# knowhunger/go-libp2p-pubsub

Hardware: AMD Instinct MI355X
Metric: peer-topic score updates/s + msg deliveries/s @1M peers, 1-8 GPUs, %HBM BW (higher is better)
Workload: dtype f64; 1 GPU; cfg3: 1M peers x 8 topics, full P1-P7 refreshScores()+score() per DecayInterval, connectSome d=6 overlay, spam-test topic params; peers_per_gpu=1000000, topics=8, pairs_per_gpu=11999954, records_per_gpu=95999632, parallelism=observers range-sharded, 1 shard(s), no exchange

## Files before the change

### go-libp2p-pubsub_amd/csrc/gsx_device.h

```cpp
#pragma once

#include <hip/hip_runtime.h>
#include <stdint.h>

namespace gsx {

struct DevTopicParams {
    double topic_weight;
    double w1, cap1;
    int64_t q1;
    double inv_q1;
    double w2, d2, cap2;
    double w3, d3, cap3, thr3;
    int64_t win3, act3;
    double w3b, d3b;
    double w4, d4;
    int32_t scored;
    int32_t pad;
};

__host__ __device__ __forceinline__ double q1_inverse(int64_t q1) { return q1 > 0 ? 1.0 / (double)q1 : 0.0; }

struct DevPeerParams {
    double topic_score_cap;
    double w5;
    double w6;
    int64_t thr6;
    double w7, thr7, d7;
    double decay_to_zero;
    int64_t retain_ns;
};

constexpr int KARG_TOPICS = 8;
struct KernParams {
    DevPeerParams pp;
    DevTopicParams tp[KARG_TOPICS];
};

constexpr int TILE = 64;
constexpr int NFIELD = 5;
enum Field { FMD = 0, MMD = 1, MFP = 2, IMD = 3, GRAFT = 4 };

__host__ __device__ __forceinline__ size_t rec_index(uint64_t p, uint32_t t, uint32_t n_topics, int field) {
    return (((p / TILE) * n_topics + t) * NFIELD + field) * TILE + (p % TILE);
}
__host__ __device__ __forceinline__ size_t flag_index(uint64_t p, uint32_t t, uint32_t n_topics) {
    return ((p / TILE) * n_topics + t) * TILE + (p % TILE);
}

constexpr uint8_t ZM_ZERO = 0, ZM_MAYBE = 1;
__host__ __device__ __forceinline__ size_t zmap_index(uint64_t p, uint32_t t, uint32_t n_topics, int field) {
    return ((p / TILE) * n_topics + t) * 2 + (size_t)(field - MFP);
}
__host__ __device__ __forceinline__ size_t zmap_bytes(uint64_t n_tiles, uint32_t n_topics) {
    return ((n_tiles * n_topics * 2 + 3) / 4 + 1) * 4;
}

constexpr int PZ_APP = 0, PZ_P6 = 1, PZ_ENTRY = 4;
__host__ __device__ __forceinline__ size_t pzmap_bytes(uint64_t n_tiles) { return (n_tiles + 1) * PZ_ENTRY; }

struct DevState {
    double* rec;
    uint8_t* rflags;
    uint8_t* zmap;
    uint8_t* pzmap;
    uint8_t* pflags;
    int64_t* expire;
    double* bp;
    double* app;
    const uint32_t* ipg;
    uint32_t* ipcount;
    double* score;
    const DevTopicParams* tp;
    uint64_t n_pairs;
    uint32_t n_topics;
    int64_t last_refresh;
    uint32_t phase;
    uint32_t wb_period;
    double decay_to_zero;
    double d7;
};

constexpr uint8_t REC_IN_MESH = 0x01;
constexpr uint8_t REC_ACTIVE = 0x02;
constexpr uint8_t REC_FRESH = 0x04;
constexpr uint8_t REC_EPOCH = 0x18;
constexpr int REC_EPOCH_SHIFT = 3;
constexpr uint8_t PAIR_PRESENT = 0x01;
constexpr uint8_t PAIR_CONNECTED = 0x02;
constexpr uint8_t PAIR_EPOCH = 0x0C;
constexpr int PAIR_EPOCH_SHIFT = 2;
constexpr uint32_t IPG_NONE = 0xFFFFFFFFu;
constexpr uint32_t IPG_WL = 0x80000000u;

struct DevEvent {
    uint32_t kind;
    uint32_t topic;
    uint64_t pair;
    int64_t now_ns;
    int64_t arg;
};

struct DevSynthSpec {
    uint64_t seed;
    int64_t now;
    double fmd_max, mmd_max, mfp_max, imd_max;
    double p_in_mesh;
    int64_t graft_window;
    double bp_max, p_disc, p_abs;
    int64_t expire_jitter;
    uint32_t sybil_first;
};

constexpr uint8_t EDGE_OUTBOUND = 0x01, EDGE_DIRECT = 0x02, EDGE_GOSSIPSUB = 0x04, EDGE_FLOODSUB = 0x08,
                  EDGE_NO_PX = 0x10;
constexpr uint32_t ROUTER_FLOODSUB = 0, ROUTER_GOSSIPSUB = 1, ROUTER_RANDOMSUB = 2;
constexpr uint32_t NO_PAIR = 0xFFFFFFFFu;
constexpr uint8_t FWD_FORWARD = 0x01;
constexpr uint8_t FWD_PUBLISH = 0x02;
constexpr uint8_t FWD_RSUB_CAND = 0x04;
constexpr uint8_t FWD_SEND = 0x07;
constexpr uint8_t FWD_GIN = 0x08;
constexpr int RANDOMSUB_D = 6;
constexpr int MAX_HOPS = 64;
enum {
    STAT_DUPS = 0,
    STAT_HOP0 = 1,
    STAT_EDGE_SENDS = STAT_HOP0 + MAX_HOPS + 1,
    STAT_NEW_WORDS,
    STAT_BACKSENDS,
    STAT_REJECTED,
    STAT_IGNORED,
    STAT_GRAY,
    STAT_HALO0,
    STAT_WORDS = STAT_HALO0 + MAX_HOPS + 1
};
constexpr uint32_t HALO = 0x80000000u;
constexpr uint32_t HALO_GRAY = 0x40000000u;
constexpr uint32_t HALO_SLOT = 0x3FFFFFFFu;
constexpr int PIN_FWD_SHIFT = 29;
constexpr uint32_t MAX_RANKS = 64;
constexpr uint32_t PIN_RDROP = 1u << 28;
constexpr uint32_t PIN_NODE_MASK = PIN_RDROP - 1;
// ... 735 lines not shown
```

### go-libp2p-pubsub_amd/csrc/gsx_engine.cpp

```cpp
#include <hip/hip_runtime.h>

#include <algorithm>
#include <map>
#include <atomic>
#include <chrono>
#include <array>
#include <cmath>
#include <cstdio>
#include <cstdlib>
#include <cstring>
#include <deque>
#include <functional>
#include <string>
#include <unordered_map>
#include <unordered_set>
#include <vector>

#include "../../include/gsx.h"
#include "gsx_device.h"

namespace {

constexpr int64_t kSecond = 1000000000LL;
constexpr int64_t kTimeCacheDuration = 120 * kSecond;
constexpr uint64_t kHostScoreMax = 1u << 16;

bool invalid_number(double x) { return std::isnan(x) || std::isinf(x); }

enum { kDeliveryUnknown = 0, kDeliveryValid, kDeliveryInvalid, kDeliveryIgnored, kDeliveryThrottled };

struct RecKey {
    uint32_t obs;
    uint64_t msg;
    bool operator==(const RecKey& o) const { return obs == o.obs && msg == o.msg; }
};
struct RecKeyHash {
    size_t operator()(const RecKey& k) const {
        uint64_t x = k.msg ^ (uint64_t(k.obs) * 0x9E3779B97F4A7C15ULL);
        x ^= x >> 31;
        x *= 0xbf58476d1ce4e5b9ULL;
        x ^= x >> 29;
        return size_t(x);
    }
};
struct DeliveryRecord {
    int status = kDeliveryUnknown;
    int64_t first_seen = 0;
    int64_t validated = 0;
    bool validated_set = false;
    std::vector<uint64_t> peers;
    bool peers_nil = false;
};

}

struct gsx_engine {
    int device = 0;
    hipStream_t stream = nullptr;
    hipEvent_t ev_start = nullptr, ev_stop = nullptr, ev_staged = nullptr;
    std::string err;

    uint32_t T = 0;
    gsx_peer_score_params pp{};
    bool pp_set = false;
    gsx_thresholds th{};
    gsx_topic_score_params tp[GSX_MAX_TOPICS]{};
    bool scored[GSX_MAX_TOPICS]{};
    gsx::DevTopicParams* d_tp = nullptr;

    bool loaded = false;
    uint32_t n_nodes = 0;
    uint64_t E = 0, rs = 0, n_tiles = 0;
    int64_t last_refresh = 0;
    uint32_t phase = 0;
    uint32_t wb_period = 4;
    bool retained_possible = false;
    int64_t retain_horizon = INT64_MIN;
    uint64_t purge_launches = 0;
    std::vector<int64_t> row_ptr;
    std::vector<int32_t> col_host;
    std::vector<uint32_t> pair_obs;
    std::vector<uint32_t> ipg_host;
    std::vector<uint32_t> group_ip;
    std::vector<uint8_t> ip_wl;
    uint32_t n_groups = 0;

    double* d_rec = nullptr;
    uint8_t* d_rflags = nullptr;
    uint8_t* d_zmap = nullptr;
    uint8_t* d_pzmap = nullptr;
    void* d_tmp = nullptr;
    uint32_t* d_nbad = nullptr;
    uint8_t *d_pflags = nullptr, *d_eflags = nullptr;
    int64_t* d_expire = nullptr;
    double *d_bp = nullptr, *d_app = nullptr, *d_score = nullptr;
    uint32_t *d_ipg = nullptr, *d_ipcount = nullptr;
    int32_t* d_col = nullptr;
    int64_t* d_row_ptr = nullptr;
    uint32_t* d_rev = nullptr;
    std::vector<uint8_t> eflags_host;
    bool floodsub_peers = true;
    int64_t max_deg = 0;

    gsx_gossipsub_params gp{};
    int64_t* d_backoff = nullptr;
    uint8_t* d_bo8 = nullptr;
    uint64_t *d_ctl = nullptr, *d_resp = nullptr;
    uint8_t* d_dirty = nullptr;
    uint32_t *d_long = nullptr, *d_nlong = nullptr;
    unsigned long long* d_hbstats = nullptr;
    uint32_t* d_rngk = nullptr;
    gsx::IhaveSlot* d_ihave_slot = nullptr;
    gsx::IhaveSlot* d_ihave_unit = nullptr;
    uint8_t* d_ihave_tag = nullptr;
    uint32_t *d_work = nullptr, *d_nwork = nullptr, *d_hubwork = nullptr, *d_hubs = nullptr;
    uint8_t* d_tcnt = nullptr;
    uint16_t* d_mcount = nullptr;
    std::vector<uint32_t> hubs_host;
    std::vector<uint8_t> gossip_prev;
    uint8_t* d_gelig = nullptr;
    uint32_t ihave_round = 0;
    bool have_gossip = false;
    bool hb_clean = false;
    bool hb_tracing = false;
    uint64_t* d_tr_acc = nullptr;
    uint64_t* d_tr_hp = nullptr;
    gsx::HbState hb{};
    bool hb_active = false;
// ... 420 lines not shown
#define HIPCHK(e, call)                                                                          \
    do {                                                                                         \
        hipError_t _st = (call);                                                                 \
        if (_st != hipSuccess)                                                                   \
            return fail((e), GSX_EDEVICE, std::string(#call ": ") + hipGetErrorString(_st));    \
    } while (0)

struct ZeroBatch {
    gsx_engine* e;
    gsx::ZeroSpans z{};
    explicit ZeroBatch(gsx_engine* e_) : e(e_) {}
    int add(void* p, size_t bytes) {
        if (!p || !bytes) return GSX_OK;
        if (z.k == gsx::ZERO_SPANS)
            if (int rc = flush()) return rc;
        z.p[z.k] = static_cast<uint8_t*>(p);
        z.n[z.k++] = bytes;
        return GSX_OK;
    }
    int flush() {
        if (!z.k) return GSX_OK;
        HIPCHK(e, gsx::launch_zero_spans(z, e->stream));
        z.k = 0;
        return GSX_OK;
    }
};

int gx_busy(gsx_engine* e) {
    if (e->gxr.pending) return fail(e, GSX_ESTATE, "a sharded gossip exchange is in flight: gsx_gx_end first");
    return GSX_OK;
}

gsx::DevState dev_state(const gsx_engine* e) {
    gsx::DevState s{};
    s.rec = e->d_rec;
    s.rflags = e->d_rflags;
    s.zmap = e->d_zmap;
    s.pzmap = e->d_pzmap;
    s.pflags = e->d_pflags;
    s.expire = e->d_expire;
    s.bp = e->d_bp;
    s.app = e->d_app;
    s.ipg = e->d_ipg;
    s.ipcount = e->d_ipcount;
    s.score = e->d_score;
    s.tp = e->d_tp;
    s.n_pairs = e->E;
    s.n_topics = e->T;
    s.last_refresh = e->last_refresh;
    s.phase = e->phase;
    s.wb_period = e->wb_period;
    s.decay_to_zero = e->pp.decay_to_zero;
    s.d7 = e->pp.behaviour_penalty_decay;
    return s;
}

constexpr int64_t kRetainUnknown = INT64_MAX;
void note_retained(gsx_engine* e, int64_t bound) {
    e->retained_possible = true;
    e->retain_horizon = std::max(e->retain_horizon, bound);
}
void note_retained_events(gsx_engine* e, const std::vector<gsx_event>& evs) {
    for (const gsx_event& x : evs)
        if (x.kind == GSX_EV_REMOVE_PEER)
            note_retained(e, (int64_t)((uint64_t)x.now_ns + (uint64_t)e->pp.retain_score_ns));
}

int pzmap_mark_p6(gsx_engine* e) {
    if (!e->loaded) return GSX_OK;
    HIPCHK(e, gsx::launch_pzmap_fill(dev_state(e), gsx::PZ_P6, gsx::ZM_MAYBE, e->stream));
    return GSX_OK;
}

gsx::DevEvent dev_event(const gsx_engine* e, const gsx_event& x) {
    if (x.kind == GSX_EV_ADD_PEER) {
        const uint32_t u = e->pair_obs[x.pair];
        return gsx::DevEvent{x.kind, x.topic, x.pair, e->row_ptr[u], e->row_ptr[u + 1]};
    }
    return gsx::DevEvent{x.kind, x.topic, x.pair, x.now_ns, x.arg};
}

int materialize_all(gsx_engine* e) {
    if (!e->loaded) return GSX_OK;
    HIPCHK(e, gsx::launch_materialize(dev_state(e), e->stream));
    e->phase = 0;
    return GSX_OK;
}

gsx::DevPeerParams dev_peer_params(const gsx_engine* e) {
    gsx::DevPeerParams d{};
    d.topic_score_cap = e->pp.topic_score_cap;
    d.w5 = e->pp.app_specific_weight;
    d.w6 = e->pp.ip_colocation_factor_weight;
    d.thr6 = e->pp.ip_colocation_factor_threshold;
    d.w7 = e->pp.behaviour_penalty_weight;
    d.thr7 = e->pp.behaviour_penalty_threshold;
    d.d7 = e->pp.behaviour_penalty_decay;
    d.decay_to_zero = e->pp.decay_to_zero;
    d.retain_ns = e->pp.retain_score_ns;
    return d;
}

gsx::DevTopicParams dev_topic_params(const gsx_engine* e, uint32_t t);

gsx::KernParams kern_params(const gsx_engine* e) {
    gsx::KernParams k{};
    k.pp = dev_peer_params(e);
    for (uint32_t t = 0; t < e->T && t < (uint32_t)gsx::KARG_TOPICS; ++t) k.tp[t] = dev_topic_params(e, t);
    return k;
}

gsx::DevTopicParams dev_topic_params(const gsx_engine* e, uint32_t t) {
    gsx::DevTopicParams d{};
    const gsx_topic_score_params& p = e->tp[t];
    d.topic_weight = p.topic_weight;
    d.w1 = p.time_in_mesh_weight;
    d.cap1 = p.time_in_mesh_cap;
    d.q1 = e->scored[t] ? p.time_in_mesh_quantum_ns : 1;
    d.inv_q1 = gsx::q1_inverse(d.q1);
    d.w2 = p.first_message_deliveries_weight;
    d.d2 = p.first_message_deliveries_decay;
    d.cap2 = p.first_message_deliveries_cap;
    d.w3 = p.mesh_message_deliveries_weight;
    d.d3 = p.mesh_message_deliveries_decay;
    d.cap3 = p.mesh_message_deliveries_cap;
    d.thr3 = p.mesh_message_deliveries_threshold;
    d.win3 = p.mesh_message_deliveries_window_ns;
    d.act3 = p.mesh_message_deliveries_activation_ns;
    d.w3b = p.mesh_failure_penalty_weight;
    d.d3b = p.mesh_failure_penalty_decay;
    d.w4 = p.invalid_message_deliveries_weight;
    d.d4 = p.invalid_message_deliveries_decay;
    d.scored = e->scored[t] ? 1 : 0;
    return d;
}

int upload_topic_params(gsx_engine* e) {
    gsx::DevTopicParams h[GSX_MAX_TOPICS]{};
    for (uint32_t t = 0; t < e->T; ++t) h[t] = dev_topic_params(e, t);
    HIPCHK(e, hipMemcpyAsync(e->d_tp, h, sizeof(gsx::DevTopicParams) * GSX_MAX_TOPICS, hipMemcpyHostToDevice,
                             e->stream));
    HIPCHK(e, hipStreamSynchronize(e->stream));
    return GSX_OK;
}

void seen_release(gsx_engine* e, uint64_t* p, size_t ) {
    if (!p) return;
    auto it = e->seen_cap.find(p);
    e->seen_pool.emplace_back(it != e->seen_cap.end() ? it->second : 0, p);
}
uint64_t* seen_acquire(gsx_engine* e, size_t words) {
    size_t best = e->seen_pool.size();
    for (size_t i = 0; i < e->seen_pool.size(); ++i)
        if (e->seen_pool[i].first >= words && (best == e->seen_pool.size() || e->seen_pool[i].first < e->seen_pool[best].first))
            best = i;
    if (best < e->seen_pool.size()) {
        uint64_t* p = e->seen_pool[best].second;
        e->seen_pool.erase(e->seen_pool.begin() + (long)best);
        return p;
    }
    constexpr size_t kSlab = 4, kSlabMaxBytes = 64ull << 20;
    const size_t w = (std::max<size_t>(words, 1) + 31) & ~(size_t)31;
    const size_t n = 8 * w <= kSlabMaxBytes ? kSlab : 1;
    uint64_t* p = nullptr;
    if (hipMalloc((void**)&p, 8 * w * n) != hipSuccess) {
        if (n == 1 || hipMalloc((void**)&p, 8 * w) != hipSuccess) return nullptr;
        e->pool_slabs.push_back(p);
        e->seen_cap[p] = w;
        return p;
    }
    e->pool_slabs.push_back(p);
    for (size_t k = 0; k < n; ++k) e->seen_cap[p + k * w] = w;
    for (size_t k = 1; k < n; ++k) e->seen_pool.emplace_back(w, p + k * w);
    return p;
}
void seen_pool_free(gsx_engine* e) {
    e->seen_pool.clear();
    e->small_pool.clear();
    e->seen_cap.clear();
    for (void* x : e->pool_slabs) (void)hipFree(x);
    e->pool_slabs.clear();
}
uint8_t* small_acquire(gsx_engine* e, size_t bytes, size_t* got) {
    for (size_t i = 0; i < e->small_pool.size(); ++i)
        if (e->small_pool[i].first >= bytes && e->small_pool[i].first <= 4 * bytes + 4096) {
            uint8_t* p = e->small_pool[i].second;
// ... 1454 lines not shown
    }
    return GSX_OK;
}

int gsx_gc_deliveries(gsx_engine* e, int64_t now) {
    if (!e) return GSX_EINVAL;
    for (auto it = e->rec_queue.begin(); it != e->rec_queue.end();) {
        auto& q = it->second;
        while (!q.empty() && now > q.front().second) {
            e->recs.erase(RecKey{it->first, q.front().first});
            q.pop_front();
        }
        it = q.empty() ? e->rec_queue.erase(it) : std::next(it);
    }
    return GSX_OK;
}

int gsx_num_delivery_records(gsx_engine* e, uint64_t* out) {
    if (!e || !out) return GSX_EINVAL;
    *out = e->recs.size();
    return GSX_OK;
}

int gsx_refresh(gsx_engine* e, int64_t now) {
    if (!e) return GSX_EINVAL;
    if (!e->loaded) return fail(e, GSX_ESTATE, "no overlay loaded");
    if (int rc = fold_deferred(e)) return rc;
    int rc = flush(e);
    if (rc) return rc;
    const gsx::DevState s = dev_state(e);
    if (e->retained_possible) {
        HIPCHK(e, gsx::launch_purge(s, now, e->stream));
        ++e->purge_launches;
        if (now > e->retain_horizon) {
            e->retained_possible = false;
            e->retain_horizon = INT64_MIN;
        }
    }
    const bool region = e->t_active && e->t_used < e->t_max;
    HIPCHK(e, hipEventRecord(region ? e->tev[2 * e->t_used] : e->ev_start, e->stream));
    HIPCHK(e, rescore_all(e, s, now, true));
    HIPCHK(e, hipEventRecord(region ? e->tev[2 * e->t_used + 1] : e->ev_stop, e->stream));
    if (region) ++e->t_used;
    e->timed = !region;
    e->scores_exact();
    e->state_changed();
    e->last_refresh = now;
    e->phase = e->phase + 1 >= e->wb_period ? 0 : e->phase + 1;
    return GSX_OK;
}

int gsx_set_decay_writeback(gsx_engine* e, uint32_t k) {
    if (!e) return GSX_EINVAL;
    if (k != 1 && k != 2 && k != 4) return fail(e, GSX_EINVAL, "decay write-back period must be 1, 2 or 4");
    if (int rc = gx_busy(e)) return rc;
    if (int rc = fold_deferred(e)) return rc;
    if (int rc = flush(e)) return rc;
    if (int rc = materialize_all(e)) return rc;
    e->wb_period = k;
    return GSX_OK;
}

int gsx_last_refresh_ms(gsx_engine* e, float* ms) {
    if (!e || !ms) return GSX_EINVAL;
    if (!e->timed) return fail(e, GSX_ESTATE, "no refresh timed yet");
    HIPCHK(e, hipEventSynchronize(e->ev_stop));
    HIPCHK(e, hipEventElapsedTime(ms, e->ev_start, e->ev_stop));
    return GSX_OK;
}

int gsx_timing_begin(gsx_engine* e, uint32_t max_launches) {
    if (!e || max_launches == 0) return GSX_EINVAL;
    while (e->tev.size() < 2 * (size_t)max_launches) {
        hipEvent_t ev;
        HIPCHK(e, hipEventCreate(&ev));
        e->tev.push_back(ev);
    }
    e->t_max = max_launches;
    e->t_used = 0;
    e->t_active = true;
    return GSX_OK;
}

int gsx_timing_end(gsx_engine* e, double* total_ms, double* min_ms, double* max_ms, uint32_t* n) {
    if (!e || !total_ms || !n) return GSX_EINVAL;
    if (!e->t_active) return fail(e, GSX_ESTATE, "gsx_timing_begin not called");
    e->t_active = false;
    double sum = 0, lo = 0, hi = 0;
    for (uint32_t i = 0; i < e->t_used; ++i) {
        HIPCHK(e, hipEventSynchronize(e->tev[2 * i + 1]));
        float ms = 0;
        HIPCHK(e, hipEventElapsedTime(&ms, e->tev[2 * i], e->tev[2 * i + 1]));
        sum += ms;
        lo = i == 0 ? ms : std::min(lo, (double)ms);
        hi = i == 0 ? ms : std::max(hi, (double)ms);
    }
    *total_ms = sum;
    *n = e->t_used;
    if (min_ms) *min_ms = lo;
    if (max_ms) *max_ms = hi;
    return GSX_OK;
}

int gsx_scores(gsx_engine* e, double* out, size_t n) {
    if (!e || (n && !out)) return GSX_EINVAL;
    if (!e->loaded) return fail(e, GSX_ESTATE, "no overlay loaded");
    if (n != e->E) return fail(e, GSX_EINVAL, "score buffer size != pairs");
// ... 5022 lines not shown
```

### go-libp2p-pubsub_amd/csrc/gsx_kernels.hip

```cpp
#include "gsx_ops.h"

namespace gsx {


__device__ __forceinline__ uint64_t wave_uniform(uint64_t x) {
    return (uint64_t)__builtin_amdgcn_readfirstlane((uint32_t)x) |
           (uint64_t)__builtin_amdgcn_readfirstlane((uint32_t)(x >> 32)) << 32;
}

constexpr uint32_t ZM_MFP_BITS = 0x00FFu, ZM_IMD_BITS = 0xFF00u;
__device__ __forceinline__ uint32_t zmap_pair(const uint8_t* zmap, uint64_t o) {
    const uint32_t w = reinterpret_cast<const uint32_t*>(zmap)[o >> 2];
    return __builtin_amdgcn_readfirstlane((w >> ((uint32_t)(o & 2) * 8)) & 0xFFFFu);
}

template <int TT, bool REFRESH>
__global__ __launch_bounds__(256) void k_refresh_score(DevState s, KernParams kp, int64_t now,
                                                       const uint8_t* __restrict__ only,
                                                       const uint8_t* __restrict__ only2,
                                                       const unsigned long long* __restrict__ gate) {
    const uint64_t p = (uint64_t)blockIdx.x * 256u + threadIdx.x;
    if (p >= s.n_pairs) return;
    if (!REFRESH && gate && gate[0] + gate[1] == 0) return;
    if (!REFRESH && only && (!only[p] || (only2 && !only2[p]))) return;
    const int T = TT > 0 ? TT : (int)s.n_topics;
    const uint64_t lane = p % TILE;
    const uint64_t wtile = wave_uniform(p / TILE);
    const uint64_t zoff = wtile * (uint64_t)T * 2;
    uint32_t zm[TT > 0 ? TT : 1];
    if constexpr (TT > 0) {
#pragma unroll
        for (int t = 0; t < TT; ++t) zm[t] = zmap_pair(s.zmap, zoff + 2 * t);
    }
    const uint32_t pz = __builtin_amdgcn_readfirstlane(reinterpret_cast<const uint32_t*>(s.pzmap)[wtile]);
    const bool app_maybe = (pz >> (8 * PZ_APP)) & 0xFFu;
    const bool p6_maybe = !REFRESH || ((pz >> (8 * PZ_P6)) & 0xFFu);
    const uint8_t st = s.pflags[p];
    if (!(st & PAIR_PRESENT)) {
        s.score[p] = 0.0;
        return;
    }
    const DevPeerParams& pp = kp.pp;
    double p5 = 0.0;
    if (app_maybe) p5 = s.app[p];
    const bool conn = REFRESH && (st & PAIR_CONNECTED);
    const uint32_t phase = s.phase;
    const bool wb = REFRESH && phase + 1 >= s.wb_period;
    const bool lag = st & PAIR_CONNECTED;
    const uint8_t keep_conn = (uint8_t)~(REC_FRESH | (wb ? REC_EPOCH : 0));
    double* const tile = s.rec + (p / TILE) * (uint64_t)T * (NFIELD * TILE) + lane;
    uint8_t* const ftile = s.rflags + (p / TILE) * (uint64_t)T * TILE + lane;
    double score = 0.0;
    auto topic_step = [&](int t, const DevTopicParams& tp, double fmd, double mmd, double mfp, double imd,
                          int64_t graft, uint8_t fl, uint32_t zmt) {
        double* const r = tile + (uint64_t)t * (NFIELD * TILE);
        const double fmd0 = fmd, mmd0 = mmd, mfp0 = mfp, imd0 = imd;
        const uint32_t nd = (lag ? (phase - ((uint32_t)fl >> REC_EPOCH_SHIFT)) & 3u : 0u) + (conn ? 1u : 0u);
        const uint32_t nd0 = __builtin_amdgcn_readfirstlane(nd);
        auto decay_all = [&]() {
            fmd = decay(fmd, tp.d2, pp.decay_to_zero);
            mmd = decay(mmd, tp.d3, pp.decay_to_zero);
            mfp = decay(mfp, tp.d3b, pp.decay_to_zero);
            imd = decay(imd, tp.d4, pp.decay_to_zero);
        };
        if (__ballot(nd != nd0) == 0) {
            for (uint32_t i = 0; i < nd0; ++i) decay_all();
        } else {
            for (uint32_t i = 0; i < nd; ++i) decay_all();
        }
        if (wb) {
            if (conn && __double_as_longlong(fmd) != __double_as_longlong(fmd0)) __builtin_nontemporal_store(fmd, r + FMD * TILE);
            if (conn && __double_as_longlong(mmd) != __double_as_longlong(mmd0)) __builtin_nontemporal_store(mmd, r + MMD * TILE);
            if (conn && __double_as_longlong(mfp) != __double_as_longlong(mfp0)) __builtin_nontemporal_store(mfp, r + MFP * TILE);
            if (conn && __double_as_longlong(imd) != __double_as_longlong(imd0)) __builtin_nontemporal_store(imd, r + IMD * TILE);
        }
        const bool in_mesh = fl & REC_IN_MESH;
        int64_t mt = 0;
        if (conn) {
            mt = in_mesh ? now - graft : 0;
            const uint8_t nf = (uint8_t)((fl & keep_conn) | ((in_mesh && mt > tp.act3) ? REC_ACTIVE : 0));
            if (nf != fl) ftile[t * TILE] = nf;
            fl = nf;
        } else if (in_mesh && !(fl & REC_FRESH)) {
            mt = s.last_refresh - graft;
        }
        if constexpr (REFRESH) {
            if (zmt && __ballot(1) == ~0ull) {
                uint8_t* const zb = s.zmap + zoff + 2 * t;
                const bool z3 = (zmt & ZM_MFP_BITS) && __ballot(__double_as_longlong(mfp) != 0) == 0;
                const bool z4 = (zmt & ZM_IMD_BITS) && __ballot(__double_as_longlong(imd) != 0) == 0;
                if (z3 && !wb && __double_as_longlong(mfp0) != 0) r[MFP * TILE] = 0.0;
                if (z4 && !wb && __double_as_longlong(imd0) != 0) r[IMD * TILE] = 0.0;
                if (z3 && lane == 0) zb[0] = ZM_ZERO;
                if (z4 && lane == 0) zb[1] = ZM_ZERO;
            }
        }
        score += topic_score(tp, fl, mt, fmd, mmd, mfp, imd);
    };
    if constexpr (TT > 0) {
        double fmd[TT], mmd[TT], mfp[TT], imd[TT];
        int64_t gr[TT];
        uint8_t fl[TT];
#pragma unroll
        for (int t = 0; t < TT; ++t) {
            if (!kp.tp[t].scored) continue;
            const double* const r = tile + (uint64_t)t * (NFIELD * TILE);
            fmd[t] = __builtin_nontemporal_load(r + FMD * TILE);
            mmd[t] = __builtin_nontemporal_load(r + MMD * TILE);
            mfp[t] = (zm[t] & ZM_MFP_BITS) ? __builtin_nontemporal_load(r + MFP * TILE) : 0.0;
            imd[t] = (zm[t] & ZM_IMD_BITS) ? __builtin_nontemporal_load(r + IMD * TILE) : 0.0;
            fl[t] = ftile[t * TILE];
            gr[t] = (TT > 1 || (fl[t] & REC_IN_MESH))
                        ? __builtin_nontemporal_load(reinterpret_cast<const int64_t*>(r) + GRAFT * TILE)
                        : 0;
        }
#pragma unroll
        for (int t = 0; t < TT; ++t) {
            if (!kp.tp[t].scored) continue;
            topic_step(t, kp.tp[t], fmd[t], mmd[t], mfp[t], imd[t], gr[t], fl[t], zm[t]);
        }
    } else {
        for (int t = 0; t < T; ++t) {
            const DevTopicParams& tp = s.tp[t];
            if (!tp.scored) continue;
            const double* const r = tile + (uint64_t)t * (NFIELD * TILE);
            const uint32_t zmt = zmap_pair(s.zmap, zoff + 2 * t);
            const uint8_t fl = ftile[t * TILE];
            const int64_t graft = (fl & REC_IN_MESH) ? reinterpret_cast<const int64_t*>(r)[GRAFT * TILE] : 0;
            const double fmd = __builtin_nontemporal_load(r + FMD * TILE), mmd = __builtin_nontemporal_load(r + MMD * TILE);
            const double mfp = (zmt & ZM_MFP_BITS) ? __builtin_nontemporal_load(r + MFP * TILE) : 0.0;
            const double imd = (zmt & ZM_IMD_BITS) ? __builtin_nontemporal_load(r + IMD * TILE) : 0.0;
            topic_step(t, tp, fmd, mmd, mfp, imd, graft, fl, zmt);
        }
    }
    const double bp0 = s.bp[p];
    double bp = bp0;
    const uint32_t nb = (lag ? (phase - ((uint32_t)st >> PAIR_EPOCH_SHIFT)) & 3u : 0u) + (conn ? 1u : 0u);
    const uint32_t nb0 = __builtin_amdgcn_readfirstlane(nb);
    if (__ballot(nb != nb0) == 0) {
        for (uint32_t i = 0; i < nb0; ++i) bp = decay(bp, pp.d7, pp.decay_to_zero);
    } else {
        for (uint32_t i = 0; i < nb; ++i) bp = decay(bp, pp.d7, pp.decay_to_zero);
    }
    if (wb && conn) {
        if (__double_as_longlong(bp) != __double_as_longlong(bp0)) s.bp[p] = bp;
        if (st & PAIR_EPOCH) s.pflags[p] = st & ~PAIR_EPOCH;
    }
    double p6 = 0.0;
    const bool p6_read = pp.w6 != 0.0 && p6_maybe;
    if (p6_read) p6 = ip_colocation(s, pp, p);
    s.score[p] = score_tail_vals(pp, score, p5, p6, bp);
    if constexpr (REFRESH) {
        if ((app_maybe || p6_read) && __ballot(1) == ~0ull) {
            uint8_t* const pzb = s.pzmap + wtile * PZ_ENTRY;
            const bool z5 = app_maybe && __ballot(__double_as_longlong(p5) != 0) == 0;
            const bool z6 = p6_read && __ballot(__double_as_longlong(p6) != 0) == 0;
            if (z5 && lane == 0) pzb[PZ_APP] = ZM_ZERO;
            if (z6 && lane == 0) pzb[PZ_P6] = ZM_ZERO;
        }
    }
}

__global__ __launch_bounds__(256) void k_purge(DevState s, int64_t now) {
    const uint64_t p = (uint64_t)blockIdx.x * 256u + threadIdx.x;
    if (p >= s.n_pairs) return;
    const uint8_t st = s.pflags[p];
    if ((st & (PAIR_PRESENT | PAIR_CONNECTED)) != PAIR_PRESENT) return;
    if (!(now > s.expire[p])) return;
    s.pflags[p] = 0;
    const uint2 g = reinterpret_cast<const uint2*>(s.ipg)[p];
    if (g.x != IPG_NONE) atomicSub(&s.ipcount[g.x & ~IPG_WL], 1u);
    if (g.y != IPG_NONE && g.y != g.x) atomicSub(&s.ipcount[g.y & ~IPG_WL], 1u);
}


__device__ __forceinline__ void apply_event(const DevState& s, const DevPeerParams& pp, const DevEvent& e) {
    switch (e.kind) {
    case 1: ev_add_peer(s, pp, e.pair, (uint64_t)e.now_ns, (uint64_t)e.arg); break;
    case 2: ev_remove_peer(s, pp, e.pair, e.now_ns); break;
    case 3: ev_graft(s, e.pair, e.topic, e.now_ns); break;
    case 4: ev_prune(s, e.pair, e.topic); break;
    case 5: ev_first(s, e.pair, e.topic); break;
    case 6: ev_mesh(s, e.pair, e.topic); break;
    case 7: ev_invalid(s, e.pair, e.topic); break;
    case 8: ev_penalty(s, e.pair, e.arg); break;
    case 9:
        if (e.arg != 0) pzmap_mark(s, e.pair, PZ_APP);
        s.app[e.pair] = __longlong_as_double((long long)e.arg);
        break;
    default: break;
    }
}

__global__ __launch_bounds__(64) void k_apply_events(DevState s, DevPeerParams pp, const DevEvent* __restrict__ ev,
                                                     const uint32_t* __restrict__ group_off, uint32_t n_groups) {
// ... 278 lines not shown
hipError_t launch_mark_rows(const int64_t* row_ptr, const uint32_t* obs, uint32_t n, uint8_t* mask, uint8_t val,
                            hipStream_t st) {
    if (n == 0) return hipSuccess;
    hipLaunchKernelGGL(k_mark_rows, dim3(std::min<uint32_t>((n + 3) / 4, 4096)), dim3(256), 0, st, row_ptr, obs, n, mask,
                       val);
    return hipGetLastError();
}

hipError_t launch_apply_events(const DevState& s, const DevPeerParams& pp, const DevEvent* ev,
                               const uint32_t* group_off, uint32_t n_groups, hipStream_t st) {
    if (n_groups == 0) return hipSuccess;
    hipLaunchKernelGGL(k_apply_events, dim3(blocks_for(n_groups, 64)), dim3(64), 0, st, s, pp, ev, group_off,
                       n_groups);
    return hipGetLastError();
}

hipError_t launch_dropin(const DevState& s, const DevPeerParams& pp, const DevEvent* ev, const uint32_t* goff,
                         uint32_t n_groups, const uint32_t* obs, uint32_t n_obs, const uint64_t* prs, uint32_t n_prs,
                         const int64_t* row_ptr, double* hscore, uint32_t* flag, uint32_t tag, hipStream_t st) {
    hipLaunchKernelGGL(k_dropin, dim3(1), dim3(n_obs ? 1024 : 256), 0, st, s, pp, ev, goff, n_groups, obs, n_obs, prs,
                       n_prs, row_ptr, hscore, flag, tag);
    return hipGetLastError();
}

hipError_t launch_gather_scores(const double* score, const uint64_t* pairs, uint64_t n, double* out, hipStream_t st) {
    if (n == 0) return hipSuccess;
    const uint64_t b = (n + 255) / 256;
    hipLaunchKernelGGL(k_gather_scores, dim3((unsigned)(b < 4096 ? b : 4096)), dim3(256), 0, st, score, pairs, n, out);
    return hipGetLastError();
}

hipError_t launch_recap(const DevState& s, uint32_t topic, double cap2, double cap3, hipStream_t st) {
    if (s.n_pairs == 0) return hipSuccess;
    hipLaunchKernelGGL(k_recap, dim3(blocks_for(s.n_pairs, 256)), dim3(256), 0, st, s, topic, cap2, cap3);
    return hipGetLastError();
}

__global__ __launch_bounds__(256) void k_materialize(DevState s) {
    const uint64_t p = (uint64_t)blockIdx.x * 256u + threadIdx.x;
    const uint32_t t = blockIdx.y;
    if (p >= s.n_pairs) return;
    const size_t fi = flag_index(p, t, s.n_topics);
    const uint8_t fl = s.rflags[fi];
    const uint32_t k = rec_pend(s, s.pflags[p], fl, s.tp[t]);
    if (k) rec_store_decayed(s, p, t, k);
    if (fl & REC_EPOCH) s.rflags[fi] = fl & ~REC_EPOCH;
}
__global__ __launch_bounds__(256) void k_materialize_pairs(DevState s) {
    const uint64_t p = (uint64_t)blockIdx.x * 256u + threadIdx.x;
    if (p >= s.n_pairs) return;
    const uint8_t st = s.pflags[p];
    const uint32_t k = bp_pend(s, st);
    if (k) {
        const double o = s.bp[p], v = bp_decay(o, s.d7, s.decay_to_zero, k);
        if (__double_as_longlong(v) != __double_as_longlong(o)) s.bp[p] = v;
    }
    if (st & PAIR_EPOCH) s.pflags[p] = st & ~PAIR_EPOCH;
}
hipError_t launch_materialize(const DevState& s, hipStream_t st) {
    if (s.n_pairs == 0) return hipSuccess;
    hipLaunchKernelGGL(k_materialize, dim3(blocks_for(s.n_pairs, 256), s.n_topics), dim3(256), 0, st, s);
    hipLaunchKernelGGL(k_materialize_pairs, dim3(blocks_for(s.n_pairs, 256)), dim3(256), 0, st, s);
    return hipGetLastError();
}

__global__ __launch_bounds__(256) void k_pair_export(DevState s, uint8_t* __restrict__ pf, double* __restrict__ bp) {
    const uint64_t p = (uint64_t)blockIdx.x * 256u + threadIdx.x;
    if (p >= s.n_pairs) return;
    const uint8_t st = s.pflags[p];
    if (pf) pf[p] = st & ~PAIR_EPOCH;
    if (bp) bp[p] = bp_read(s, p, st);
}
hipError_t launch_pair_export(const DevState& s, uint8_t* pflags, double* bp, hipStream_t st) {
    if (s.n_pairs == 0) return hipSuccess;
    hipLaunchKernelGGL(k_pair_export, dim3(blocks_for(s.n_pairs, 256)), dim3(256), 0, st, s, pflags, bp);
    return hipGetLastError();
}

hipError_t launch_rebuild_ipcount(const DevState& s, uint32_t n_groups_ip, hipStream_t st) {
    hipError_t e = hipMemsetAsync(s.ipcount, 0, sizeof(uint32_t) * (n_groups_ip ? n_groups_ip : 1), st);
    if (e != hipSuccess || s.n_pairs == 0) return e;
    hipLaunchKernelGGL(k_rebuild_ipcount, dim3(blocks_for(s.n_pairs, 256)), dim3(256), 0, st, s);
    return hipGetLastError();
}

hipError_t launch_synthesize(const DevState& s, const int32_t* col, const DevSynthSpec& spec, hipStream_t st) {
    if (s.n_pairs == 0) return hipSuccess;
    const unsigned nb = blocks_for(s.n_pairs, 256);
    hipLaunchKernelGGL(k_synth_records, dim3(nb, s.n_topics), dim3(256), 0, st, s, col, spec);
    hipLaunchKernelGGL(k_synth_pairs, dim3(nb), dim3(256), 0, st, s, spec);
    return hipGetLastError();
}

hipError_t launch_tile_field(const DevState& s, int field, const void* src, hipStream_t st) {
    if (s.n_pairs == 0) return hipSuccess;
    hipLaunchKernelGGL(k_tile_field, dim3(blocks_for(s.n_pairs, 256), s.n_topics), dim3(256), 0, st, s, field, src);
    return hipGetLastError();
}

hipError_t launch_untile_field(const DevState& s, int field, void* dst, hipStream_t st) {
    if (s.n_pairs == 0) return hipSuccess;
    hipLaunchKernelGGL(k_untile_field, dim3(blocks_for(s.n_pairs, 256), s.n_topics), dim3(256), 0, st, s, field, dst);
    return hipGetLastError();
}

hipError_t launch_mesh_time_export(const DevState& s, int64_t* dst, hipStream_t st) {
    if (s.n_pairs == 0) return hipSuccess;
// ... 52 lines not shown
```

### go-libp2p-pubsub_amd/csrc/gsx_ops.h

```cpp
#pragma once

#include "gsx_device.h"

namespace gsx {


__device__ __forceinline__ double ip_colocation(const DevState& s, const DevPeerParams& pp, uint64_t p) {
    const uint2 g = reinterpret_cast<const uint2*>(s.ipg)[p];
    double result = 0.0;
    const uint32_t gs[2] = {g.x, g.y};
#pragma unroll
    for (int k = 0; k < 2; ++k) {
        const uint32_t id = gs[k];
        if (id == IPG_NONE || (id & IPG_WL)) continue;
        const int64_t peers_in_ip = (int64_t)s.ipcount[id];
        if (peers_in_ip > pp.thr6) {
            const double surpluss = (double)(peers_in_ip - pp.thr6);
            result += surpluss * surpluss;
        }
    }
    return result;
}

__device__ __forceinline__ double score_tail_vals(const DevPeerParams& pp, double score, double p5, double p6,
// ... 18 lines not shown
constexpr int64_t DIV_Q1_BOUND = 1ll << 50;

__host__ __device__ __forceinline__ int64_t div_q1(int64_t mt, int64_t q1, double inv) {
    if (inv != 0.0 && (uint64_t)mt + (uint64_t)DIV_Q1_BOUND - 1u < 2u * (uint64_t)DIV_Q1_BOUND - 1u) {
        const double est = (double)mt * inv;
        const double sum = est + 6755399441055744.0;
#if defined(__HIP_DEVICE_COMPILE__)
        const uint64_t bits = (uint64_t)__double_as_longlong(sum);
#else
        uint64_t bits;
        __builtin_memcpy(&bits, &sum, sizeof bits);
#endif
        int64_t n = (int64_t)(bits & ((1ull << 52) - 1)) - (1ll << 51);
        const int64_t r = (int64_t)((uint64_t)mt - (uint64_t)n * (uint64_t)q1);
        const bool neg = mt < 0;
        const bool up = neg ? r > 0 : r >= q1;
        const bool down = neg ? r <= -q1 : r < 0;
        n += (int64_t)up - (int64_t)down;
        return n;
    }
    return mt / q1;
}

__device__ __forceinline__ double topic_score(const DevTopicParams& tp, uint8_t fl, int64_t mesh_time, double fmd,
                                              double mmd, double mfp, double imd) {
    double ts = 0.0;
    if (fl & REC_IN_MESH) {
        double p1 = (double)div_q1(mesh_time, tp.q1, tp.inv_q1);
        if (p1 > tp.cap1) p1 = tp.cap1;
        ts += p1 * tp.w1;
    }
    const double p2 = fmd;
    ts += p2 * tp.w2;
    if (fl & REC_ACTIVE) {
        if (mmd < tp.thr3) {
            const double deficit = tp.thr3 - mmd;
            const double p3 = deficit * deficit;
            ts += p3 * tp.w3;
        }
    }
    const double p3b = mfp;
    ts += p3b * tp.w3b;
    const double p4 = (imd * imd);
    ts += p4 * tp.w4;
    return ts * tp.topic_weight;
}

__device__ __forceinline__ int64_t mesh_time_of(const DevState& s, uint8_t fl, uint64_t p, uint32_t t) {
    if (!(fl & REC_IN_MESH) || (fl & REC_FRESH)) return 0;
    const int64_t graft = reinterpret_cast<const int64_t*>(s.rec)[rec_index(p, t, s.n_topics, GRAFT)];
    return s.last_refresh - graft;
}

__device__ __forceinline__ double decay(double x, double d, double dtz) {
    x *= d;
    return x < dtz ? 0.0 : x;
}

__device__ __forceinline__ void zmap_mark(const DevState& s, uint64_t p, uint32_t t, int field) {
    s.zmap[zmap_index(p, t, s.n_topics, field)] = ZM_MAYBE;
}

__device__ __forceinline__ void pzmap_mark(const DevState& s, uint64_t p, int which) {
    s.pzmap[(p / TILE) * PZ_ENTRY + which] = ZM_MAYBE;
}
__device__ __forceinline__ void pzmap_mark_row(const DevState& s, uint64_t lo, uint64_t hi) {
    if (hi > s.n_pairs) hi = s.n_pairs;
    if (lo >= hi) return;
    for (uint64_t tile = lo / TILE; tile <= (hi - 1) / TILE; ++tile) s.pzmap[tile * PZ_ENTRY + PZ_P6] = ZM_MAYBE;
}

struct RecVals {
    double fmd, mmd, mfp, imd;
};

__device__ __forceinline__ uint32_t rec_pend(const DevState& s, uint8_t st, uint8_t fl, const DevTopicParams& tp) {
    return ((st & PAIR_CONNECTED) && tp.scored) ? ((s.phase - ((uint32_t)fl >> REC_EPOCH_SHIFT)) & 3u) : 0u;
}

__device__ __forceinline__ void rec_decay(RecVals& v, const DevTopicParams& tp, double dtz, uint32_t k) {
    for (uint32_t i = 0; i < k; ++i) {
        v.fmd = decay(v.fmd, tp.d2, dtz);
        v.mmd = decay(v.mmd, tp.d3, dtz);
        v.mfp = decay(v.mfp, tp.d3b, dtz);
        v.imd = decay(v.imd, tp.d4, dtz);
    }
}

__device__ __forceinline__ RecVals rec_read(const DevState& s, uint64_t p, uint32_t t, uint8_t st, uint8_t fl) {
    const size_t b = rec_index(p, t, s.n_topics, FMD);
    RecVals v = {s.rec[b + FMD * TILE], s.rec[b + MMD * TILE], s.rec[b + MFP * TILE], s.rec[b + IMD * TILE]};
    rec_decay(v, s.tp[t], s.decay_to_zero, rec_pend(s, st, fl, s.tp[t]));
    return v;
}
__device__ __forceinline__ RecVals rec_read(const DevState& s, uint64_t p, uint32_t t) {
    return rec_read(s, p, t, s.pflags[p], s.rflags[flag_index(p, t, s.n_topics)]);
}

__device__ __forceinline__ void rec_store_decayed(const DevState& s, uint64_t p, uint32_t t, uint32_t k) {
    const size_t b = rec_index(p, t, s.n_topics, FMD);
    const RecVals o = {s.rec[b + FMD * TILE], s.rec[b + MMD * TILE], s.rec[b + MFP * TILE], s.rec[b + IMD * TILE]};
    RecVals v = o;
    rec_decay(v, s.tp[t], s.decay_to_zero, k);
    if (__double_as_longlong(v.fmd) != __double_as_longlong(o.fmd)) s.rec[b + FMD * TILE] = v.fmd;
    if (__double_as_longlong(v.mmd) != __double_as_longlong(o.mmd)) s.rec[b + MMD * TILE] = v.mmd;
    if (__double_as_longlong(v.mfp) != __double_as_longlong(o.mfp)) {
        if (__double_as_longlong(v.mfp) != 0) zmap_mark(s, p, t, MFP);
        s.rec[b + MFP * TILE] = v.mfp;
    }
    if (__double_as_longlong(v.imd) != __double_as_longlong(o.imd)) {
        if (__double_as_longlong(v.imd) != 0) zmap_mark(s, p, t, IMD);
        s.rec[b + IMD * TILE] = v.imd;
    }
}

__device__ __forceinline__ uint8_t rec_materialize(const DevState& s, uint64_t p, uint32_t t, uint8_t st) {
    const size_t fi = flag_index(p, t, s.n_topics);
    const uint8_t fl = s.rflags[fi];
    const uint32_t k = rec_pend(s, st, fl, s.tp[t]);
    if (k) rec_store_decayed(s, p, t, k);
    const uint8_t nf = (uint8_t)((fl & ~REC_EPOCH) | (s.phase << REC_EPOCH_SHIFT));
    if (nf != fl) s.rflags[fi] = nf;
    return nf;
}
__device__ __forceinline__ uint8_t rec_materialize(const DevState& s, uint64_t p, uint32_t t) {
    return rec_materialize(s, p, t, s.pflags[p]);
}

__device__ __forceinline__ uint32_t bp_pend(const DevState& s, uint8_t st) {
    return (st & PAIR_CONNECTED) ? ((s.phase - ((uint32_t)st >> PAIR_EPOCH_SHIFT)) & 3u) : 0u;
}

__device__ __forceinline__ double bp_decay(double bp, double d7, double dtz, uint32_t k) {
    for (uint32_t i = 0; i < k; ++i) bp = decay(bp, d7, dtz);
    return bp;
}

__device__ __forceinline__ double bp_read(const DevState& s, uint64_t p, uint8_t st) {
    return bp_decay(s.bp[p], s.d7, s.decay_to_zero, bp_pend(s, st));
}

__device__ __forceinline__ uint8_t bp_materialize(const DevState& s, uint64_t p, uint8_t st) {
    if (!(st & PAIR_CONNECTED)) return st;
    const uint32_t k = bp_pend(s, st);
    if (k) {
        const double o = s.bp[p], v = bp_decay(o, s.d7, s.decay_to_zero, k);
        if (__double_as_longlong(v) != __double_as_longlong(o)) s.bp[p] = v;
    }
    const uint8_t nf = (uint8_t)((st & ~PAIR_EPOCH) | ((s.phase & 3u) << PAIR_EPOCH_SHIFT));
    if (nf != st) s.pflags[p] = nf;
    return nf;
}

__device__ __forceinline__ double eval_pair(const DevState& s, const DevPeerParams& pp, uint64_t p) {
    const uint8_t st = s.pflags[p];
    if (!(st & PAIR_PRESENT)) return 0.0;
    double score = 0.0;
    for (uint32_t t = 0; t < s.n_topics; ++t) {
        const DevTopicParams& tp = s.tp[t];
        if (!tp.scored) continue;
        const uint8_t fl = s.rflags[flag_index(p, t, s.n_topics)];
        const RecVals v = rec_read(s, p, t, st, fl);
        score += topic_score(tp, fl, mesh_time_of(s, fl, p, t), v.fmd, v.mmd, v.mfp, v.imd);
    }
    return score_tail(s, pp, p, score, bp_read(s, p, st));
}

__device__ __forceinline__ double add_ones_capped(double x, uint32_t k, double cap) {
    while (k && !(x >= 1.0 && x < 4503599627370496.0)) {
        x = x + 1;
        --k;
        if (x > cap) return cap;
    }
    while (k) {
        const unsigned long long bits = (unsigned long long)__double_as_longlong(x);
        const double top = __longlong_as_double((long long)((((bits >> 52) & 0x7FF) + 1) << 52));
        const double gap = top - x;
        const double s = ceil(gap) - 1;
        if (s >= (double)k) {
            x = x + (double)k;
            k = 0;
        } else {
            x = x + s;
            k -= (uint32_t)s;
            x = x + 1;
            --k;
        }
        if (x > cap) return cap;
        if (!(x < 4503599627370496.0))
            while (k) {
                x = x + 1;
                --k;
                if (x > cap) return cap;
            }
    }
    return x > cap ? cap : x;
}


__device__ __forceinline__ void ipcount_add(const DevState& s, uint64_t p, int delta) {
    const uint2 g = reinterpret_cast<const uint2*>(s.ipg)[p];
    if (g.x != IPG_NONE) s.ipcount[g.x & ~IPG_WL] += (uint32_t)delta;
    if (g.y != IPG_NONE && g.y != g.x) s.ipcount[g.y & ~IPG_WL] += (uint32_t)delta;
}

__device__ __forceinline__ bool scored_topic(const DevState& s, uint64_t p, uint32_t topic) {
    return (s.pflags[p] & PAIR_PRESENT) && topic < s.n_topics && s.tp[topic].scored;
}

__device__ inline void ev_add_peer(const DevState& s, const DevPeerParams& pp, uint64_t p, uint64_t row_lo,
                                   uint64_t row_hi) {
    const uint8_t st = s.pflags[p];
    const uint8_t ep = (uint8_t)(s.phase << REC_EPOCH_SHIFT);
    if (!(st & PAIR_PRESENT)) {
        for (uint32_t t = 0; t < s.n_topics; ++t) {
            const size_t b = rec_index(p, t, s.n_topics, FMD);
            for (int f = 0; f < NFIELD; ++f) s.rec[b + f * TILE] = 0.0;
            s.rflags[flag_index(p, t, s.n_topics)] = ep;
        }
        s.bp[p] = 0.0;
        s.expire[p] = 0;
        ipcount_add(s, p, +1);
        const uint2 g = reinterpret_cast<const uint2*>(s.ipg)[p];
        const bool over_x = g.x != IPG_NONE && !(g.x & IPG_WL) && (int64_t)s.ipcount[g.x] > pp.thr6;
        const bool over_y = g.y != IPG_NONE && !(g.y & IPG_WL) && (int64_t)s.ipcount[g.y] > pp.thr6;
        if (over_x || over_y) {
            pzmap_mark(s, p, PZ_P6);
            pzmap_mark_row(s, row_lo, row_hi);
        }
    } else if (!(st & PAIR_CONNECTED)) {
        for (uint32_t t = 0; t < s.n_topics; ++t) {
            const size_t fi = flag_index(p, t, s.n_topics);
            const uint8_t fl = s.rflags[fi];
            if ((fl & REC_EPOCH) != ep) s.rflags[fi] = (uint8_t)((fl & ~REC_EPOCH) | ep);
        }
    }
    if (!(st & PAIR_PRESENT) || !(st & PAIR_CONNECTED))
        s.pflags[p] = (uint8_t)(PAIR_PRESENT | PAIR_CONNECTED | ((s.phase & 3u) << PAIR_EPOCH_SHIFT));
}

__device__ inline void ev_remove_peer(const DevState& s, const DevPeerParams& pp, uint64_t p, int64_t now) {
    const uint8_t st = s.pflags[p];
    if (!(st & PAIR_PRESENT)) return;
    if (eval_pair(s, pp, p) > 0) {
        ipcount_add(s, p, -1);
        bp_materialize(s, p, st);
        s.pflags[p] = 0;
        return;
    }
    for (uint32_t t = 0; t < s.n_topics; ++t) {
        const DevTopicParams& tp = s.tp[t];
        if (!tp.scored) continue;
        const size_t b = rec_index(p, t, s.n_topics, FMD);
        const size_t fi = flag_index(p, t, s.n_topics);
        const uint8_t fl = rec_materialize(s, p, t, st);
        s.rec[b + FMD * TILE] = 0.0;
        const double threshold = tp.thr3;
        const double mmd = s.rec[b + MMD * TILE];
        if ((fl & REC_IN_MESH) && (fl & REC_ACTIVE) && mmd < threshold) {
            const double deficit = threshold - mmd;
            zmap_mark(s, p, t, MFP);
            s.rec[b + MFP * TILE] = s.rec[b + MFP * TILE] + deficit * deficit;
        }
        s.rflags[fi] = fl & ~(REC_IN_MESH | REC_FRESH);
    }
    bp_materialize(s, p, st);
    s.pflags[p] = PAIR_PRESENT;
    s.expire[p] = now + pp.retain_ns;
}

__device__ inline void ev_graft(const DevState& s, uint64_t p, uint32_t topic, int64_t now) {
    if (!scored_topic(s, p, topic)) return;
    reinterpret_cast<int64_t*>(s.rec)[rec_index(p, topic, s.n_topics, GRAFT)] = now;
    const size_t fi = flag_index(p, topic, s.n_topics);
    s.rflags[fi] = (uint8_t)((s.rflags[fi] & REC_EPOCH) | REC_IN_MESH | REC_FRESH);
}

__device__ inline void ev_prune(const DevState& s, uint64_t p, uint32_t topic) {
    if (!scored_topic(s, p, topic)) return;
    const size_t b = rec_index(p, topic, s.n_topics, FMD);
    const size_t fi = flag_index(p, topic, s.n_topics);
    const uint8_t fl = rec_materialize(s, p, topic);
    const double threshold = s.tp[topic].thr3;
    const double mmd = s.rec[b + MMD * TILE];
    if ((fl & REC_ACTIVE) && mmd < threshold) {
        const double deficit = threshold - mmd;
        zmap_mark(s, p, topic, MFP);
        s.rec[b + MFP * TILE] = s.rec[b + MFP * TILE] + deficit * deficit;
    }
    s.rflags[fi] = fl & ~(REC_IN_MESH | REC_FRESH);
}
// ... 104 lines not shown
```

Measured before the change: 145.9 billion peer-topic score updates/s.

## Widen decay epoch to 16 phases and chain multiplies before the zero threshold

Widens the per-record and per-pair epoch fields from 2 to 4 bits and raises the default write-back period from 4 to 16. Decayed counters are therefore written back to HBM less often, cutting store traffic during refresh. When every decay factor is in (0,1) and decay_to_zero is positive, pending decays are applied as a run of multiplies with a single threshold check at the end instead of one clamp per step. The chained form may differ from per-step clamping in edge cases, and lagging records now replay up to 16 decay steps when read.

```diff
diff --git a/go-libp2p-pubsub_amd/csrc/gsx_device.h b/go-libp2p-pubsub_amd/csrc/gsx_device.h
--- a/go-libp2p-pubsub_amd/csrc/gsx_device.h
+++ b/go-libp2p-pubsub_amd/csrc/gsx_device.h
@@ -16,7 +16,7 @@
     double w3b, d3b;
     double w4, d4;
     int32_t scored;
-    int32_t pad;
+    int32_t chain_ok;
 };
 
 __host__ __device__ __forceinline__ double q1_inverse(int64_t q1) { return q1 > 0 ? 1.0 / (double)q1 : 0.0; }
@@ -29,7 +29,11 @@
     double w7, thr7, d7;
     double decay_to_zero;
     int64_t retain_ns;
-};
+    int32_t dtz_ok;
+    int32_t bp_chain_ok;
+};
+
+__host__ __device__ __forceinline__ bool decay_chain_ok(double d, double dtz) { return d > 0.0 && d < 1.0 && dtz > 0.0; }
 
 constexpr int KARG_TOPICS = 8;
 struct KernParams {
@@ -79,16 +83,20 @@
     uint32_t wb_period;
     double decay_to_zero;
     double d7;
+    uint32_t dtz_ok;
+    uint32_t bp_chain_ok;
 };
 
 constexpr uint8_t REC_IN_MESH = 0x01;
 constexpr uint8_t REC_ACTIVE = 0x02;
 constexpr uint8_t REC_FRESH = 0x04;
-constexpr uint8_t REC_EPOCH = 0x18;
+constexpr uint32_t MAX_WB_PERIOD = 16;
+constexpr uint32_t EPOCH_MASK = MAX_WB_PERIOD - 1;
+constexpr uint8_t REC_EPOCH = 0x78;
 constexpr int REC_EPOCH_SHIFT = 3;
 constexpr uint8_t PAIR_PRESENT = 0x01;
 constexpr uint8_t PAIR_CONNECTED = 0x02;
-constexpr uint8_t PAIR_EPOCH = 0x0C;
+constexpr uint8_t PAIR_EPOCH = 0x3C;
 constexpr int PAIR_EPOCH_SHIFT = 2;
 constexpr uint32_t IPG_NONE = 0xFFFFFFFFu;
 constexpr uint32_t IPG_WL = 0x80000000u;
diff --git a/go-libp2p-pubsub_amd/csrc/gsx_engine.cpp b/go-libp2p-pubsub_amd/csrc/gsx_engine.cpp
--- a/go-libp2p-pubsub_amd/csrc/gsx_engine.cpp
+++ b/go-libp2p-pubsub_amd/csrc/gsx_engine.cpp
@@ -73,7 +73,7 @@
     uint64_t E = 0, rs = 0, n_tiles = 0;
     int64_t last_refresh = 0;
     uint32_t phase = 0;
-    uint32_t wb_period = 4;
+    uint32_t wb_period = gsx::MAX_WB_PERIOD;
     bool retained_possible = false;
     int64_t retain_horizon = INT64_MIN;
     uint64_t purge_launches = 0;
@@ -600,6 +600,8 @@
     s.wb_period = e->wb_period;
     s.decay_to_zero = e->pp.decay_to_zero;
     s.d7 = e->pp.behaviour_penalty_decay;
+    s.dtz_ok = e->pp.decay_to_zero > 0 ? 1u : 0u;
+    s.bp_chain_ok = gsx::decay_chain_ok(s.d7, s.decay_to_zero) ? 1u : 0u;
     return s;
 }
 
@@ -646,6 +648,8 @@
     d.d7 = e->pp.behaviour_penalty_decay;
     d.decay_to_zero = e->pp.decay_to_zero;
     d.retain_ns = e->pp.retain_score_ns;
+    d.dtz_ok = d.decay_to_zero > 0 ? 1 : 0;
+    d.bp_chain_ok = gsx::decay_chain_ok(d.d7, d.decay_to_zero) ? 1 : 0;
     return d;
 }
 
@@ -680,6 +684,7 @@
     d.w4 = p.invalid_message_deliveries_weight;
     d.d4 = p.invalid_message_deliveries_decay;
     d.scored = e->scored[t] ? 1 : 0;
+    d.chain_ok = (d.d2 > 0 && d.d2 < 1 && d.d3 > 0 && d.d3 < 1 && d.d3b > 0 && d.d3b < 1 && d.d4 > 0 && d.d4 < 1) ? 1 : 0;
     return d;
 }
 
@@ -2240,7 +2245,8 @@
 
 int gsx_set_decay_writeback(gsx_engine* e, uint32_t k) {
     if (!e) return GSX_EINVAL;
-    if (k != 1 && k != 2 && k != 4) return fail(e, GSX_EINVAL, "decay write-back period must be 1, 2 or 4");
+    if (k != 1 && k != 2 && k != 4 && k != gsx::MAX_WB_PERIOD)
+        return fail(e, GSX_EINVAL, "decay write-back period must be 1, 2, 4 or 16");
     if (int rc = gx_busy(e)) return rc;
     if (int rc = fold_deferred(e)) return rc;
     if (int rc = flush(e)) return rc;
diff --git a/go-libp2p-pubsub_amd/csrc/gsx_kernels.hip b/go-libp2p-pubsub_amd/csrc/gsx_kernels.hip
--- a/go-libp2p-pubsub_amd/csrc/gsx_kernels.hip
+++ b/go-libp2p-pubsub_amd/csrc/gsx_kernels.hip
@@ -55,19 +55,16 @@
                           int64_t graft, uint8_t fl, uint32_t zmt) {
         double* const r = tile + (uint64_t)t * (NFIELD * TILE);
         const double fmd0 = fmd, mmd0 = mmd, mfp0 = mfp, imd0 = imd;
-        const uint32_t nd = (lag ? (phase - ((uint32_t)fl >> REC_EPOCH_SHIFT)) & 3u : 0u) + (conn ? 1u : 0u);
+        const uint32_t nd = (lag ? (phase - ((uint32_t)fl >> REC_EPOCH_SHIFT)) & EPOCH_MASK : 0u) + (conn ? 1u : 0u);
         const uint32_t nd0 = __builtin_amdgcn_readfirstlane(nd);
-        auto decay_all = [&]() {
-            fmd = decay(fmd, tp.d2, pp.decay_to_zero);
-            mmd = decay(mmd, tp.d3, pp.decay_to_zero);
-            mfp = decay(mfp, tp.d3b, pp.decay_to_zero);
-            imd = decay(imd, tp.d4, pp.decay_to_zero);
-        };
+        const bool chain = tp.chain_ok && pp.dtz_ok;
+        RecVals v = {fmd, mmd, mfp, imd};
         if (__ballot(nd != nd0) == 0) {
-            for (uint32_t i = 0; i < nd0; ++i) decay_all();
+            rec_decay(v, tp, pp.decay_to_zero, nd0, chain);
         } else {
-            for (uint32_t i = 0; i < nd; ++i) decay_all();
-        }
+            rec_decay(v, tp, pp.decay_to_zero, nd, chain);
+        }
+        fmd = v.fmd, mmd = v.mmd, mfp = v.mfp, imd = v.imd;
         if (wb) {
             if (conn && __double_as_longlong(fmd) != __double_as_longlong(fmd0)) __builtin_nontemporal_store(fmd, r + FMD * TILE);
             if (conn && __double_as_longlong(mmd) != __double_as_longlong(mmd0)) __builtin_nontemporal_store(mmd, r + MMD * TILE);
@@ -135,12 +132,12 @@
     }
     const double bp0 = s.bp[p];
     double bp = bp0;
-    const uint32_t nb = (lag ? (phase - ((uint32_t)st >> PAIR_EPOCH_SHIFT)) & 3u : 0u) + (conn ? 1u : 0u);
+    const uint32_t nb = (lag ? (phase - ((uint32_t)st >> PAIR_EPOCH_SHIFT)) & EPOCH_MASK : 0u) + (conn ? 1u : 0u);
     const uint32_t nb0 = __builtin_amdgcn_readfirstlane(nb);
     if (__ballot(nb != nb0) == 0) {
-        for (uint32_t i = 0; i < nb0; ++i) bp = decay(bp, pp.d7, pp.decay_to_zero);
+        bp = bp_decay(bp, pp.d7, pp.decay_to_zero, nb0, pp.bp_chain_ok);
     } else {
-        for (uint32_t i = 0; i < nb; ++i) bp = decay(bp, pp.d7, pp.decay_to_zero);
+        bp = bp_decay(bp, pp.d7, pp.decay_to_zero, nb, pp.bp_chain_ok);
     }
     if (wb && conn) {
         if (__double_as_longlong(bp) != __double_as_longlong(bp0)) s.bp[p] = bp;
@@ -525,7 +522,7 @@
     const uint8_t st = s.pflags[p];
     const uint32_t k = bp_pend(s, st);
     if (k) {
-        const double o = s.bp[p], v = bp_decay(o, s.d7, s.decay_to_zero, k);
+        const double o = s.bp[p], v = bp_decay(o, s.d7, s.decay_to_zero, k, s.bp_chain_ok);
         if (__double_as_longlong(v) != __double_as_longlong(o)) s.bp[p] = v;
     }
     if (st & PAIR_EPOCH) s.pflags[p] = st & ~PAIR_EPOCH;
diff --git a/go-libp2p-pubsub_amd/csrc/gsx_ops.h b/go-libp2p-pubsub_amd/csrc/gsx_ops.h
--- a/go-libp2p-pubsub_amd/csrc/gsx_ops.h
+++ b/go-libp2p-pubsub_amd/csrc/gsx_ops.h
@@ -94,8 +94,14 @@
     return s.last_refresh - graft;
 }
 
-__device__ __forceinline__ double decay(double x, double d, double dtz) {
+__host__ __device__ __forceinline__ double decay(double x, double d, double dtz) {
     x *= d;
+    return x < dtz ? 0.0 : x;
+}
+
+__host__ __device__ __forceinline__ double decay_chain(double x, double d, double dtz, uint32_t k) {
+    if (k == 0) return x;
+    for (uint32_t i = 0; i < k; ++i) x *= d;
     return x < dtz ? 0.0 : x;
 }
 
@@ -117,10 +123,24 @@
 };
 
 __device__ __forceinline__ uint32_t rec_pend(const DevState& s, uint8_t st, uint8_t fl, const DevTopicParams& tp) {
-    return ((st & PAIR_CONNECTED) && tp.scored) ? ((s.phase - ((uint32_t)fl >> REC_EPOCH_SHIFT)) & 3u) : 0u;
-}
-
-__device__ __forceinline__ void rec_decay(RecVals& v, const DevTopicParams& tp, double dtz, uint32_t k) {
+    return ((st & PAIR_CONNECTED) && tp.scored) ? ((s.phase - ((uint32_t)fl >> REC_EPOCH_SHIFT)) & EPOCH_MASK) : 0u;
+}
+
+__device__ __forceinline__ void rec_decay(RecVals& v, const DevTopicParams& tp, double dtz, uint32_t k, bool chain) {
+    if (chain) {
+        if (k == 0) return;
+        for (uint32_t i = 0; i < k; ++i) {
+            v.fmd *= tp.d2;
+            v.mmd *= tp.d3;
+            v.mfp *= tp.d3b;
+            v.imd *= tp.d4;
+        }
+        v.fmd = v.fmd < dtz ? 0.0 : v.fmd;
+        v.mmd = v.mmd < dtz ? 0.0 : v.mmd;
+        v.mfp = v.mfp < dtz ? 0.0 : v.mfp;
+        v.imd = v.imd < dtz ? 0.0 : v.imd;
+        return;
+    }
     for (uint32_t i = 0; i < k; ++i) {
         v.fmd = decay(v.fmd, tp.d2, dtz);
         v.mmd = decay(v.mmd, tp.d3, dtz);
@@ -132,7 +152,7 @@
 __device__ __forceinline__ RecVals rec_read(const DevState& s, uint64_t p, uint32_t t, uint8_t st, uint8_t fl) {
     const size_t b = rec_index(p, t, s.n_topics, FMD);
     RecVals v = {s.rec[b + FMD * TILE], s.rec[b + MMD * TILE], s.rec[b + MFP * TILE], s.rec[b + IMD * TILE]};
-    rec_decay(v, s.tp[t], s.decay_to_zero, rec_pend(s, st, fl, s.tp[t]));
+    rec_decay(v, s.tp[t], s.decay_to_zero, rec_pend(s, st, fl, s.tp[t]), s.tp[t].chain_ok && s.dtz_ok);
     return v;
 }
 __device__ __forceinline__ RecVals rec_read(const DevState& s, uint64_t p, uint32_t t) {
@@ -143,7 +163,7 @@
     const size_t b = rec_index(p, t, s.n_topics, FMD);
     const RecVals o = {s.rec[b + FMD * TILE], s.rec[b + MMD * TILE], s.rec[b + MFP * TILE], s.rec[b + IMD * TILE]};
     RecVals v = o;
-    rec_decay(v, s.tp[t], s.decay_to_zero, k);
+    rec_decay(v, s.tp[t], s.decay_to_zero, k, s.tp[t].chain_ok && s.dtz_ok);
     if (__double_as_longlong(v.fmd) != __double_as_longlong(o.fmd)) s.rec[b + FMD * TILE] = v.fmd;
     if (__double_as_longlong(v.mmd) != __double_as_longlong(o.mmd)) s.rec[b + MMD * TILE] = v.mmd;
     if (__double_as_longlong(v.mfp) != __double_as_longlong(o.mfp)) {
@@ -170,26 +190,27 @@
 }
 
 __device__ __forceinline__ uint32_t bp_pend(const DevState& s, uint8_t st) {
-    return (st & PAIR_CONNECTED) ? ((s.phase - ((uint32_t)st >> PAIR_EPOCH_SHIFT)) & 3u) : 0u;
-}
-
-__device__ __forceinline__ double bp_decay(double bp, double d7, double dtz, uint32_t k) {
+    return (st & PAIR_CONNECTED) ? ((s.phase - ((uint32_t)st >> PAIR_EPOCH_SHIFT)) & EPOCH_MASK) : 0u;
+}
+
+__device__ __forceinline__ double bp_decay(double bp, double d7, double dtz, uint32_t k, bool chain) {
+    if (chain) return decay_chain(bp, d7, dtz, k);
     for (uint32_t i = 0; i < k; ++i) bp = decay(bp, d7, dtz);
     return bp;
 }
 
 __device__ __forceinline__ double bp_read(const DevState& s, uint64_t p, uint8_t st) {
-    return bp_decay(s.bp[p], s.d7, s.decay_to_zero, bp_pend(s, st));
+    return bp_decay(s.bp[p], s.d7, s.decay_to_zero, bp_pend(s, st), s.bp_chain_ok);
 }
 
 __device__ __forceinline__ uint8_t bp_materialize(const DevState& s, uint64_t p, uint8_t st) {
     if (!(st & PAIR_CONNECTED)) return st;
     const uint32_t k = bp_pend(s, st);
     if (k) {
-        const double o = s.bp[p], v = bp_decay(o, s.d7, s.decay_to_zero, k);
+        const double o = s.bp[p], v = bp_decay(o, s.d7, s.decay_to_zero, k, s.bp_chain_ok);
         if (__double_as_longlong(v) != __double_as_longlong(o)) s.bp[p] = v;
     }
-    const uint8_t nf = (uint8_t)((st & ~PAIR_EPOCH) | ((s.phase & 3u) << PAIR_EPOCH_SHIFT));
+    const uint8_t nf = (uint8_t)((st & ~PAIR_EPOCH) | ((s.phase & EPOCH_MASK) << PAIR_EPOCH_SHIFT));
     if (nf != st) s.pflags[p] = nf;
     return nf;
 }
@@ -278,7 +299,7 @@
         }
     }
     if (!(st & PAIR_PRESENT) || !(st & PAIR_CONNECTED))
-        s.pflags[p] = (uint8_t)(PAIR_PRESENT | PAIR_CONNECTED | ((s.phase & 3u) << PAIR_EPOCH_SHIFT));
+        s.pflags[p] = (uint8_t)(PAIR_PRESENT | PAIR_CONNECTED | ((s.phase & EPOCH_MASK) << PAIR_EPOCH_SHIFT));
 }
 
 __device__ inline void ev_remove_peer(const DevState& s, const DevPeerParams& pp, uint64_t p, int64_t now) {
```

After: 148.0 billion peer-topic score updates/s, median of 6. +1.4%, better.
